# ylab-hi/BINARY

Measured on AMD Instinct MI355X. Metric: interval-overlap queries/s, higher is better.
Workload: dtype u32

## Files before the change

### binary_amd/csrc/build.hip

```cpp
#include "common.h"
#include "wave_device.h"

namespace bivx {
namespace {

constexpr int kThreads = 256;

__device__ __forceinline__ uint32_t len_bin(uint32_t low, uint32_t high, uint32_t &len) {
  len = high >= low ? high - low : 0u;
  return len == 0 ? 0u : 32u - (uint32_t)__clz((int)len);
}


constexpr uint32_t kStatsLdsEntries = 3300;
#ifndef BIVX_STATS_PARTS
#define BIVX_STATS_PARTS 64
#endif
constexpr uint32_t kStatsAutoParts = BIVX_STATS_PARTS;
#ifndef BIVX_STATS_THREADS
#define BIVX_STATS_THREADS 1024
#endif
constexpr int kStatsThreads = BIVX_STATS_THREADS;
#ifndef BIVX_STATS_UNROLL
#define BIVX_STATS_UNROLL 8
// ... 533 lines not shown
            const uint32_t g = atomicAdd(ngaps, 1u);
            if (g < gap_cap) gaps[g] = Gap{g0, gc, gv, 0u};
          }
        } else {
          for (uint32_t c = lane; c < gc; c += kWave) table[g0 + c] = gv;
        }
      }
    };
    cooperative(cnt > kInlineFill, e0, cnt, val);
    cooperative(tcnt > kInlineFill, t0, tcnt, tval);
  }
}

__global__ __launch_bounds__(kThreads) void k_fill_gaps(const Gap *__restrict__ gaps, const uint32_t *__restrict__ ngaps,
                                                        uint32_t gap_cap, uint32_t *__restrict__ table) {
  const uint32_t ng = min(*ngaps, gap_cap);
  const uint32_t t = blockIdx.x * kThreads + threadIdx.x, nt = gridDim.x * kThreads;
  for (uint32_t g = 0; g < ng; ++g) {
    const Gap gp = gaps[g];
    for (uint32_t c = t; c < gp.count; c += nt) table[gp.first + c] = gp.value;
  }
}

__global__ __launch_bounds__(kThreads) void k_max_cell(uint32_t *__restrict__ table, size_t nentries,
                                                       uint32_t *__restrict__ out) {
  uint32_t m = 0;
  auto diff = [](uint32_t a, uint32_t b) { return b > a ? b - a : 0u; };
  const size_t n4 = nentries ? (nentries - 1) / 4 : 0;
  const uint4 *t4 = reinterpret_cast<const uint4 *>(table);
  const size_t stride = (size_t)gridDim.x * kThreads;
  for (size_t g = (size_t)blockIdx.x * kThreads + threadIdx.x; g < n4; g += 2 * stride) {
    const size_t g2 = g + stride;
    const bool two = g2 < n4;
    const uint4 v = t4[g];
    const uint32_t nx = table[4 * g + 4];
    uint4 w = make_uint4(0u, 0u, 0u, 0u);
    uint32_t nw = 0;
    if (two) {
      w = t4[g2];
      nw = table[4 * g2 + 4];
    }
    m = max(max(m, diff(v.x, v.y)), max(max(diff(v.y, v.z), diff(v.z, v.w)), diff(v.w, nx)));
    if (two) m = max(max(m, diff(w.x, w.y)), max(max(diff(w.y, w.z), diff(w.z, w.w)), diff(w.w, nw)));
  }
  if (blockIdx.x == 0)
    for (size_t i = 4 * n4 + threadIdx.x; i + 1 < nentries; i += kThreads) m = max(m, diff(table[i], table[i + 1]));
  if (blockIdx.x == 0 && threadIdx.x < 3) table[nentries + threadIdx.x] = 0xFFFFFFFFu;
  block_max_to(m, out);
}

__global__ __launch_bounds__(kThreads) void k_self_queries(const uint2 *__restrict__ se, const SegDesc *__restrict__ seg,
                                                           const uint32_t *__restrict__ seg_chrom, uint32_t nseg, size_t n,
                                                           uint32_t *__restrict__ qchrom, uint32_t *__restrict__ qlow,
                                                           uint32_t *__restrict__ qhigh) {
  const size_t i = (size_t)blockIdx.x * kThreads + threadIdx.x;
  if (i >= n) return;
  uint32_t lo = 0, hi = nseg;
  while (hi - lo > 1) {
    const uint32_t m = (lo + hi) >> 1;
    if ((size_t)seg[m].begin <= i) lo = m; else hi = m;
  }
  const uint2 e = se[i];
  qchrom[i] = seg_chrom[lo];
  qlow[i] = e.x;
  qhigh[i] = e.y;
}

inline unsigned grid_for(size_t n, int per_block, unsigned cap = 0) {
  size_t nb = (n + (size_t)per_block - 1) / (size_t)per_block;
  if (nb < 1) nb = 1;
  if (cap && nb > cap) nb = cap;
// ... 112 lines not shown
  for (int shift = first_shift; shift < nbits || iota; shift += kRadixBits) {
    if (!(hist0_ready && shift == first_shift))
      hipLaunchKernelGGL(k_radix_hist, dim3(nblocks), dim3(kSortThreads), 0, s, *keys, n, shift, hist, nblocks);
    hipLaunchKernelGGL(k_radix_rows, dim3(kRadix), dim3(kThreads), 0, s, hist, offs, totals, nblocks);
    if (iota)
      hipLaunchKernelGGL(k_radix_scatter<true>, dim3(nblocks), dim3(kSortThreads), 0, s, *keys, *vals, *keys_alt,
                         *vals_alt, n, shift, offs, totals, nblocks);
    else
      hipLaunchKernelGGL(k_radix_scatter<false>, dim3(nblocks), dim3(kSortThreads), 0, s, *keys, *vals, *keys_alt,
                         *vals_alt, n, shift, offs, totals, nblocks);
    BIVX_HIP(hipGetLastError());
    iota = false;
    uint32_t *t = *keys; *keys = *keys_alt; *keys_alt = t;
    t = *vals; *vals = *vals_alt; *vals_alt = t;
  }
  return 0;
}

size_t finalize_gap_capacity(uint64_t nentries, uint32_t nseg) { return (size_t)(nentries / kCoopMax) + 2u * nseg + 64u; }
size_t finalize_gap_bytes(uint64_t nentries, uint32_t nseg) { return finalize_gap_capacity(nentries, nseg) * sizeof(Gap); }

int launch_finalize(const uint32_t *d_keys, const uint32_t *d_ids, const uint32_t *d_low, const uint32_t *d_high,
                    const SegDesc *d_seg, const uint2 *d_segkey, uint32_t nseg, uint2 *d_se, uint2 *d_rec,
                    uint32_t *d_table, uint64_t nentries, void *d_gaps, uint32_t *d_ngaps, uint32_t *d_max_cell,
                    size_t n, hipStream_t s) {
  if (n == 0 || nseg == 0) return 0;
  const uint32_t nchunks = grid_for(n, kThreads * kFinSlots);
  const unsigned grid = ((nchunks + 7u) / 8u) * 8u;
  const uint32_t cap = (uint32_t)finalize_gap_capacity(nentries, nseg);
  Gap *gaps = static_cast<Gap *>(d_gaps);
  if (d_keys)
    hipLaunchKernelGGL(k_finalize<true>, dim3(grid), dim3(kThreads), 0, s, d_keys, d_ids, d_low, d_high, d_seg, d_segkey, nseg,
                       d_se, d_rec, d_table, gaps, d_ngaps, cap, n, nchunks);
  else
    hipLaunchKernelGGL(k_finalize<false>, dim3(grid), dim3(kThreads), 0, s, d_keys, d_ids, d_low, d_high, d_seg, d_segkey,
                       nseg, d_se, d_rec, d_table, gaps, d_ngaps, cap, n, nchunks);
  hipLaunchKernelGGL(k_fill_gaps, dim3(256), dim3(kThreads), 0, s, gaps, d_ngaps, cap, d_table);
  hipLaunchKernelGGL(k_max_cell, dim3(grid_for(nentries, kThreads * 8, 512)), dim3(kThreads), 0, s, d_table, (size_t)nentries,
                     d_max_cell);
  BIVX_HIP(hipGetLastError());
  return 0;
}

int launch_self_queries(const uint2 *d_se, const SegDesc *d_seg, const uint32_t *d_seg_chrom, uint32_t nseg, size_t n,
                        uint32_t *d_qchrom, uint32_t *d_qlow, uint32_t *d_qhigh, hipStream_t s) {
  if (n == 0 || nseg == 0) return 0;
  hipLaunchKernelGGL(k_self_queries, dim3(grid_for(n, kThreads)), dim3(kThreads), 0, s, d_se, d_seg, d_seg_chrom, nseg, n,
                     d_qchrom, d_qlow, d_qhigh);
  BIVX_HIP(hipGetLastError());
  return 0;
}

int launch_gather_intervals(const uint32_t *d_chrom, const uint32_t *d_low, const uint32_t *d_high,
                            const uint32_t *d_ids, size_t n, size_t n_intervals, uint32_t *d_c, uint32_t *d_l,
                            uint32_t *d_h, hipStream_t s) {
  if (n == 0) return 0;
  hipLaunchKernelGGL(k_gather_intervals, dim3(grid_for(n, kThreads)), dim3(kThreads), 0, s, d_chrom, d_low, d_high,
                     d_ids, n, n_intervals, d_c, d_l, d_h);
  BIVX_HIP(hipGetLastError());
  return 0;
}

// ... 2 lines not shown
```

### binary_amd/csrc/capi.hip

```cpp
#include <algorithm>
#include <atomic>
#include <chrono>
#include <cstdarg>
#include <cstdio>
#include <cstdlib>
#include <condition_variable>
#include <cstring>
#include <map>
#include <mutex>
#include <new>
#include <unordered_map>
#include <unordered_set>
#include <vector>

#include "common.h"

namespace bivx {

static thread_local char g_err[512] = "";

void set_error(const char *fmt, ...) {
  va_list ap;
  va_start(ap, fmt);
  vsnprintf(g_err, sizeof(g_err), fmt, ap);
// ... 16 lines not shown
    void *p = nullptr;
    size_t cap = 0;
  };
  DevBuf b_se, b_table, b_seg;
  DevBuf b_keys[2], b_ids[2];
  DevBuf b_misc, b_radix, b_scalar, b_segof;
  DevBuf b_astats;
  bool astats_ready = false;
  size_t astats_n = 0;
  hipEvent_t astats_ev = nullptr;
  uint32_t *h_scalars = nullptr;
  void *h_stage = nullptr;
  size_t h_stage_cap = 0;
  std::vector<hipEvent_t> ev_pending, ev_free;
  mutable DevBuf b_selfq;
  mutable bool selfq_valid = false;
  mutable std::mutex self_mutex;
  uint32_t *d_seg_chrom = nullptr;
  bool built = false;
  uint2 *d_se = nullptr;
  uint2 *d_rec = nullptr;
  uint32_t *d_id = nullptr;
  uint32_t *d_table = nullptr;
  SegDesc *d_seg = nullptr;
  uint2 *d_chrom_rng = nullptr;
  uint32_t nchrom = 0, nseg = 0, ntypes = 1;
  std::vector<uint32_t> max_segs;
  uint64_t nentries = 0;
  uint32_t max_cell = 0;
  uint32_t max_window = 0;
  uint32_t order_shift = 0;
  size_t built_n = 0;
  double build_ms = 0.0;
  struct Workspace {
    void *p = nullptr;
    bool needs_reset = false;
    void *self_p = nullptr;
    size_t self_cap = 0;
  };
  mutable std::mutex ws_mutex;
  mutable std::unordered_map<hipStream_t, Workspace> ws_of_stream;
  mutable std::unordered_set<hipStream_t> reader_streams;
  uint32_t *h_err = nullptr;
  uint32_t *d_err = nullptr;
  mutable std::atomic<uint64_t> errors_reported{0};
  mutable std::mutex cache_mutex;
// ... 96 lines not shown
    if (!p) BIVX_HIP(dev_malloc(&p, bytes));
    ptrs.emplace_back(p, bytes);
    *out = static_cast<T *>(p);
    return 0;
  }
  void release(void *p) {
    for (auto &q : ptrs)
      if (q.first == p) q.first = nullptr;
  }
};

void drop_block_cache(const bivx_index *idx) {
  std::lock_guard<std::mutex> lock(idx->cache_mutex);
  for (auto &kv : idx->cache_free) (void)hipFree(kv.second);
  idx->cache_free.clear();
  idx->cache_bytes = 0;
}

void free_built(bivx_index *idx) {
  idx->d_se = nullptr;
  idx->d_rec = nullptr;
  idx->d_id = nullptr;
  idx->d_table = nullptr;
  idx->d_seg = nullptr;
  idx->d_chrom_rng = nullptr;
  idx->nchrom = idx->nseg = 0;
  idx->ntypes = 1;
  idx->max_segs.clear();
  idx->nentries = 0;
  idx->built = false;
  idx->selfq_valid = false;
}

void release_build_blocks(bivx_index *idx) {
  for (bivx_index::DevBuf *b : {&idx->b_se, &idx->b_table, &idx->b_seg, &idx->b_keys[0],
                                &idx->b_keys[1], &idx->b_ids[0], &idx->b_ids[1], &idx->b_misc, &idx->b_radix, &idx->b_scalar, &idx->b_segof, &idx->b_selfq, &idx->b_astats}) {
    (void)hipFree(b->p);
    b->p = nullptr;
    b->cap = 0;
  }
}

int ensure_block(bivx_index::DevBuf &b, size_t bytes) {
  if (bytes <= b.cap && b.p) return 0;
  (void)hipFree(b.p);
  b.p = nullptr;
// ... 297 lines not shown
      (void)packed_span;
    }
  }
  return 0;
}

int bits_for(uint32_t maxval) {
  int b = 0;
  while (maxval) {
    ++b;
    maxval >>= 1;
  }
  return b;
}

static thread_local uint32_t *g_lane_d_err = nullptr;

IndexView view_of(const bivx_index *idx, uint32_t svtype = 0) {
  IndexView v;
  v.se = idx->d_se;
  v.rec = idx->d_rec;
  v.id = idx->d_id;
  v.table = idx->d_table;
  v.seg = idx->d_seg;
  const uint32_t row = svtype < idx->ntypes ? svtype : idx->ntypes;
  v.chrom_rng = idx->d_chrom_rng + (size_t)row * idx->nchrom;
  v.nchrom = idx->nchrom;
  v.nseg = idx->nseg;
  v.max_segs = row < idx->max_segs.size() ? idx->max_segs[row] : 0;
  v.nslots = idx->built_n < 0xFFFFFFFFull ? (uint32_t)idx->built_n : 0xFFFFFFFFu;
  v.max_cell = idx->max_cell;
  v.max_window = idx->max_window;
  v.order_shift = idx->order_shift;
  v.flt_kind = BIVX_FILTER_NONE;
  v.flt_dist = 0;
  v.flt_strand = 0;
  v.flt_qaux = nullptr;
  v.flt_iaux = nullptr;
  v.err = g_lane_d_err ? g_lane_d_err : idx->d_err;
  return v;
}

int report_device_errors(const bivx_index *idx, const char *who, uint32_t *block = nullptr) {
  uint32_t *e = block ? block : idx->h_err;
  if (__atomic_load_n(&e[kErrTimeout], __ATOMIC_RELAXED) == 0 && __atomic_load_n(&e[kErrWorkspace], __ATOMIC_RELAXED) == 0)
    return 0;
// ... 493 lines not shown
    const uint32_t *cs = plan.chrom_seg.data() + (size_t)c * ntypes;
    rng[c] = make_uint2(cs[0], cs[ntypes] - cs[0]);
    max_segs[0] = std::max(max_segs[0], cs[ntypes] - cs[0]);
    for (uint32_t t = 1; t < ntypes; ++t) {
      rng[(size_t)t * nchrom + c] = make_uint2(cs[t], cs[t + 1] - cs[t]);
      max_segs[t] = std::max(max_segs[t], cs[t + 1] - cs[t]);
    }
  }
  if (!plan.bin2seg.empty()) std::memcpy(hm + off_b2s, plan.bin2seg.data(), plan.bin2seg.size() * sizeof(uint32_t));
  BIVX_HIP(hipMemcpyAsync(dm, hm, meta_bytes, hipMemcpyHostToDevice, s));

  uint32_t max_cell = 0, order_shift = 0;
  if (n) {
    for (int k = 0; k < 2; ++k) {
      BIVX_TRY(ensure_block(idx->b_keys[k], n * 4));
      BIVX_TRY(ensure_block(idx->b_ids[k], (n + 2) * 4));
    }
    BIVX_TRY(ensure_block(idx->b_radix, std::max(radix_scratch_bytes(n), finalize_gap_bytes(plan.nentries, nseg))));
    const bool dense = plan.key_span <= 0xFFFFFFFFull && !std::getenv("BIVX_BUILD_TWO_STAGE");
    const size_t se_bytes = ((n + 2) * sizeof(uint2) + 255) & ~(size_t)255;
    BIVX_TRY(ensure_block(idx->b_se, 2 * se_bytes));
    idx->d_se = static_cast<uint2 *>(idx->b_se.p);
    idx->d_rec = reinterpret_cast<uint2 *>(static_cast<char *>(idx->b_se.p) + se_bytes);
    BIVX_TRY(ensure_block(idx->b_table, ((size_t)plan.nentries + 3) * 4));
    idx->d_table = static_cast<uint32_t *>(idx->b_table.p);
    auto sort_and_finalize = [&](int skip) -> int {
      uint32_t *kA = static_cast<uint32_t *>(idx->b_keys[0].p), *kB = static_cast<uint32_t *>(idx->b_keys[1].p);
      uint32_t *vA = static_cast<uint32_t *>(idx->b_ids[0].p), *vB = static_cast<uint32_t *>(idx->b_ids[1].p);
      if (dense) {
        BIVX_TRY(launch_make_keys(kBuildKeyDense, idx->d_chrom, d_type, ntypes, idx->d_low, idx->d_high, n, d_bin2seg, d_segkey,
                                  nullptr, nullptr, kA, idx->b_radix.p, s, skip));
        BIVX_TRY(radix_sort_pairs(&kA, &vA, &kB, &vB, n, bits_for((uint32_t)(plan.key_span - 1)), idx->b_radix.p, true, true, s,
                                  skip));
      } else {
        BIVX_TRY(ensure_block(idx->b_segof, n * 4));
        uint32_t *d_seg_of = static_cast<uint32_t *>(idx->b_segof.p);
        BIVX_TRY(launch_make_keys(kBuildKeyLow, idx->d_chrom, d_type, ntypes, idx->d_low, idx->d_high, n, d_bin2seg, d_segkey,
                                  nullptr, d_seg_of, kA, idx->b_radix.p, s));
        BIVX_TRY(radix_sort_pairs(&kA, &vA, &kB, &vB, n, bits_for(plan.max_low), idx->b_radix.p, true, true, s));
        if (nseg > 1) {
          BIVX_TRY(launch_make_keys(kBuildKeySegOfId, idx->d_chrom, d_type, ntypes, idx->d_low, idx->d_high, n, d_bin2seg,
                                    d_segkey, vA, d_seg_of, kA, nullptr, s));
          BIVX_TRY(radix_sort_pairs(&kA, &vA, &kB, &vB, n, bits_for(nseg - 1), idx->b_radix.p, false, false, s));
        }
      }
      idx->d_id = vA;
      BIVX_TRY(launch_finalize(dense ? kA : nullptr, idx->d_id, idx->d_low, idx->d_high, idx->d_seg, d_segkey, nseg, idx->d_se,
                               idx->d_rec, idx->d_table, plan.nentries, idx->b_radix.p, d_scalar + 3, d_scalar + 2, n, s));
      BIVX_HIP(hipMemcpyAsync(idx->h_scalars + 2, d_scalar + 2, 4, hipMemcpyDeviceToHost, s));
      return 0;
    };
    int skip = dense ? (int)plan.order_shift : 0;
    BIVX_TRY(sort_and_finalize(skip));
    if (skip > 0) {
      BIVX_HIP(hipStreamSynchronize(s));
      if (hs[2] > kCrowdedCell) {
        BIVX_HIP(hipMemsetAsync(d_scalar + 2, 0, 8, s));
        skip = 0;
        BIVX_TRY(sort_and_finalize(0));
      }
    }
    order_shift = (uint32_t)skip;
  }
  BIVX_HIP(hipStreamSynchronize(s));
  if (n) max_cell = hs[2];
  idx->nchrom = nchrom;
  idx->nseg = nseg;
  idx->ntypes = ntypes;
  idx->max_segs = std::move(max_segs);
  idx->nentries = plan.nentries;
  idx->max_cell = max_cell;
// ... 280 lines not shown
    return BIVX_E_INVALID;
  }
  BIVX_NOT_SHARDED(idx, "bivx_stream_status");
  BIVX_GUARD(idx);
  BIVX_HIP(hipStreamSynchronize(static_cast<hipStream_t>(stream)));
  return report_device_errors(idx, "bivx_stream_status");
}

int bivx_debug_corrupt_workspace(const bivx_index *idx, void *stream) {
  if (!idx) {
    set_error("bivx_debug_corrupt_workspace: null index");
    return BIVX_E_INVALID;
  }
  BIVX_NOT_SHARDED(idx, "bivx_debug_corrupt_workspace");
  BIVX_GUARD(idx);
  hipStream_t s = static_cast<hipStream_t>(stream);
  std::lock_guard<std::mutex> lock(idx->ws_mutex);
  auto it = idx->ws_of_stream.find(s);
  if (it == idx->ws_of_stream.end()) {
    set_error("bivx_debug_corrupt_workspace: no workspace for this stream yet");
    return BIVX_E_STATE;
  }
  BIVX_HIP(hipMemsetAsync(it->second.p, 0x7F, sizeof(uint32_t), s));
  return 0;
}

const char *bivx_query_kernel_name(const bivx_index *idx, size_t q, uint64_t hit_capacity, int sort_by_id,
                                   const bivx_filter *filter) {
  if (!idx || idx->sharded || !idx->built) return "";
  IndexView view;
  if (view_with_filter(idx, filter, view) != 0) return "";
  if (pipe_eligible(view, q, hit_capacity, sort_by_id != 0, false)) return "k_query_pipe";
  const bool ms = pipe_ms_eligible(view, q, hit_capacity, false);
  if (pipe_dense_eligible(view, q, hit_capacity, sort_by_id != 0, false))
    return ms ? "k_query_pipe_dense|k_query_pipe_ms" : "k_query_pipe_dense|k_query_fused";
  return ms ? "k_query_pipe_ms" : "k_query_fused";
}

int bivx_sort_hits_dev(const bivx_index *idx, const uint64_t *d_offsets, uint32_t *d_hit_ids, size_t q, void *stream) {
  if (!idx || (q && !d_offsets)) {
    set_error("bivx_sort_hits_dev: null argument");
    return BIVX_E_INVALID;
  }
  BIVX_NOT_SHARDED(idx, "bivx_sort_hits_dev");
  BIVX_GUARD(idx);
  return launch_sort_hits(d_offsets, d_hit_ids, q, ~0ull, static_cast<hipStream_t>(stream));
// ... 375 lines not shown
    set_error("bivx_query_sharded_dev: not a sharded handle (bivx_create_sharded); a single-device index answers "
              "device-resident batches with bivx_query_dev_s");
    return BIVX_E_STATE;
  }
  return sharded_query_dev(idx->sharded, qchrom, qlow, qhigh, q, sort_by_id, out);
}

int bivx_get_stats(const bivx_index *idx, bivx_stats *out) {
  if (!idx || !out) {
    set_error("bivx_get_stats: null argument");
    return BIVX_E_INVALID;
  }
  if (idx->sharded) {
    sharded_stats(idx->sharded, out);
    return 0;
  }
  memset(out, 0, sizeof(*out));
  out->n_intervals = idx->n;
  out->n_chroms = idx->nchrom;
  out->n_segments = idx->nseg;
  out->n_cells = idx->nentries;
  out->staging_bytes = (uint64_t)idx->cap * 12;
  if (idx->built)
    out->index_bytes = (uint64_t)idx->built_n * 20 + idx->nentries * 4 + (uint64_t)idx->nseg * sizeof(SegDesc) +
                       ((uint64_t)idx->nchrom + 1) * 4;
  out->build_ms = idx->build_ms;
  {
    volatile uint32_t *e = idx->h_err;
    out->prefix_timeouts = idx->errors_reported.load() + ((e[kErrTimeout] | e[kErrWorkspace]) ? 1u : 0u);
  }
  return 0;
}

}
```

### binary_amd/csrc/common.h

```cpp
#pragma once

#include <hip/hip_runtime.h>

#include <cstddef>
#include <cstdint>

#include "../../include/bivx.h"

namespace bivx {

void set_error(const char *fmt, ...) __attribute__((format(printf, 1, 2)));

#define BIVX_HIP(call)                                                                              \
  do {                                                                                              \
    hipError_t bivx_e_ = (call);                                                                    \
    if (bivx_e_ != hipSuccess) {                                                                    \
      ::bivx::set_error("%s failed: %s (%s:%d)", #call, hipGetErrorString(bivx_e_), __FILE__,       \
                        __LINE__);                                                                  \
      return BIVX_E_HIP;                                                                            \
    }                                                                                               \
  } while (0)

#define BIVX_TRY(call)              \
  do {                              \
    int bivx_rc_ = (call);          \
    if (bivx_rc_ != 0) return bivx_rc_; \
  } while (0)

constexpr int kWave = 64;
constexpr int kLenBins = 33;

struct SegDesc {
  uint32_t begin, end;
  uint32_t base, last;
  uint32_t shift;
  uint32_t table_off;
  uint32_t maxlen;
  uint32_t ncell;
};
static_assert(sizeof(SegDesc) == 32, "SegDesc layout");
constexpr uint32_t kSegPacked = 1u << 8;

struct IndexView {
  const uint2 *se;
  const uint2 *rec;
  const uint32_t *id;
  const uint32_t *table;
  const SegDesc *seg;
  const uint2 *chrom_rng;
  uint32_t nchrom;
  uint32_t nseg;
  uint32_t max_segs;
  uint32_t nslots;
  uint32_t max_cell;
  uint32_t max_window;
  uint32_t order_shift;
  uint32_t flt_kind;
  uint32_t flt_dist;
  uint32_t flt_strand;
  const uint32_t *flt_qaux;
  const uint32_t *flt_iaux;
  uint32_t *err;
};
constexpr uint32_t kErrTimeout = 0;
constexpr uint32_t kErrWorkspace = 1;
constexpr uint32_t kErrWords = 16;

struct BinStats {
  uint32_t count;
  uint32_t min_low;
  uint32_t max_low;
  uint32_t max_len;
  uint32_t n_inverted;
};

struct ShardedState;
int sharded_create(ShardedState **out, const int *devices, int ndev);
void sharded_destroy(ShardedState *st);
int sharded_num_devices(const ShardedState *st);
int sharded_device_of_chrom(const ShardedState *st, uint32_t chrom);
int sharded_append(ShardedState *st, const uint32_t *chrom, const uint32_t *low, const uint32_t *high,
                   const uint8_t *svtype, size_t n);
int sharded_clear(ShardedState *st);
size_t sharded_size(const ShardedState *st);
bool sharded_is_built(const ShardedState *st);
uint32_t sharded_num_chroms(const ShardedState *st);
// ... 27 lines not shown
int launch_bin_stats(const uint32_t *d_chrom, const uint8_t *d_type, uint32_t ntypes, const uint32_t *d_low,
                     const uint32_t *d_high, size_t n, uint32_t nparts, BinStats *d_stats, hipStream_t s);
uint32_t bin_stats_auto_parts();
int launch_bin_stats_auto(const uint32_t *d_chrom, const uint32_t *d_low, const uint32_t *d_high, size_t n, BinStats *d_stats,
                          uint32_t *d_scal, hipStream_t s);
size_t auto_stats_bytes();
int launch_init_auto_stats(void *d_block, hipStream_t s);
int launch_append_stats(const uint32_t *d_chrom, const uint32_t *d_low, const uint32_t *d_high, size_t n, uint32_t *d_out_chrom,
                        uint32_t *d_out_low, uint32_t *d_out_high, void *d_block, hipStream_t s);
int launch_max_chrom_type(const uint32_t *d_chrom, const uint8_t *d_type, size_t n, uint32_t *d_out2, hipStream_t s);
int launch_gather_u8(const uint8_t *d_src, const uint32_t *d_ids, size_t n, size_t n_src, uint8_t *d_out,
                     hipStream_t s);
enum : int { kBuildKeyDense = 0, kBuildKeyLow = 1, kBuildKeySegOfId = 2 };
int launch_make_keys(int mode, const uint32_t *d_chrom, const uint8_t *d_type, uint32_t ntypes, const uint32_t *d_low,
                     const uint32_t *d_high, size_t n, const uint32_t *d_bin2seg, const uint2 *d_segkey,
                     const uint32_t *d_ids, uint32_t *d_seg_of, uint32_t *d_keys, void *d_hist0, hipStream_t s,
                     int first_shift = 0);
size_t radix_scratch_bytes(size_t n);
int radix_sort_pairs(uint32_t **keys, uint32_t **vals, uint32_t **keys_alt, uint32_t **vals_alt, size_t n,
                     int nbits, void *d_scratch, bool vals_are_iota, bool hist0_ready, hipStream_t s, int first_shift = 0);
size_t finalize_gap_bytes(uint64_t nentries, uint32_t nseg);
int launch_finalize(const uint32_t *d_keys, const uint32_t *d_ids, const uint32_t *d_low, const uint32_t *d_high,
                    const SegDesc *d_seg, const uint2 *d_segkey, uint32_t nseg, uint2 *d_se, uint2 *d_rec,
                    uint32_t *d_table, uint64_t nentries, void *d_gaps, uint32_t *d_ngaps, uint32_t *d_max_cell,
                    size_t n, hipStream_t s);
int launch_gather_intervals(const uint32_t *d_chrom, const uint32_t *d_low, const uint32_t *d_high,
                            const uint32_t *d_ids, size_t n, size_t n_intervals, uint32_t *d_c, uint32_t *d_l,
                            uint32_t *d_h, hipStream_t s);
int launch_self_queries(const uint2 *d_se, const SegDesc *d_seg, const uint32_t *d_seg_chrom, uint32_t nseg, size_t n,
                        uint32_t *d_qchrom, uint32_t *d_qlow, uint32_t *d_qhigh, hipStream_t s);

int launch_query_tiny(const IndexView &v, const uint32_t *d_qchrom, const uint32_t *d_qlow, const uint32_t *d_qhigh,
                      size_t q, uint64_t *d_offsets, uint32_t *d_hits, uint64_t cap, hipStream_t s);
int launch_fill(const IndexView &v, const uint32_t *d_qchrom, const uint32_t *d_qlow, const uint32_t *d_qhigh,
                size_t q, const uint64_t *d_offsets, uint32_t *d_hits, hipStream_t s);
int launch_any(const IndexView &v, const uint32_t *d_qchrom, const uint32_t *d_qlow, const uint32_t *d_qhigh,
               size_t q, uint32_t *d_first, hipStream_t s);
int launch_sort_hits(const uint64_t *d_offsets, uint32_t *d_hits, size_t q, uint64_t cap, hipStream_t s,
                     const uint32_t *d_cond = nullptr, uint32_t seq = 0, uint64_t total_hint = 0);
size_t fused_workspace_bytes(size_t q);
int launch_query_fused(const IndexView &v, const uint32_t *d_qchrom, const uint32_t *d_qlow,
                       const uint32_t *d_qhigh, size_t q, uint64_t *d_offsets, uint32_t *d_hits, uint64_t cap,
                       void *d_ws, bool self_clean, bool sort_ids, hipStream_t s, uint32_t *d_counts = nullptr,
                       uint64_t *d_total = nullptr);

bool pipe_eligible(const IndexView &v, size_t q, uint64_t cap, bool sort_ids, bool unordered);
size_t pipe_queries_per_launch();
size_t pipe_ms_queries_per_launch();
// ... 21 lines not shown
```

### binary_amd/csrc/query_pipe.hip

```cpp
#include <atomic>
#include <cstdlib>

#include "prefix_device.h"
#include "query_device.h"

namespace bivx {
namespace {

#ifndef BIVX_PIPE_THREADS
#define BIVX_PIPE_THREADS 1024
#endif
constexpr int kPThreads = BIVX_PIPE_THREADS;
constexpr int kPWaves = kPThreads / kWave;
constexpr int kWorkers = kPWaves - 1;
constexpr uint32_t kPTile = kWorkers * kWave;
constexpr uint32_t kRing = 8;
#ifndef BIVX_DEFER
#define BIVX_DEFER 2
#endif
#ifndef BIVX_WSLEEP
#define BIVX_WSLEEP 16
#endif
#ifndef BIVX_SSLEEP
#define BIVX_SSLEEP 2
// ... 77 lines not shown

__device__ __forceinline__ uint32_t lds_load(const uint32_t *p) {
  return __hip_atomic_load(p, __ATOMIC_ACQUIRE, __HIP_MEMORY_SCOPE_WORKGROUP);
}
__device__ __forceinline__ void lds_store(uint32_t *p, uint32_t x) {
  __hip_atomic_store(p, x, __ATOMIC_RELEASE, __HIP_MEMORY_SCOPE_WORKGROUP);
}
__device__ __forceinline__ void lds_wait_eq(const uint32_t *p, uint32_t x) {
  while (lds_load(p) != x) __builtin_amdgcn_s_sleep(BIVX_WSLEEP);
}

__device__ __forceinline__ void stage_to_output(const uint32_t *stage, uint32_t *out, uint32_t n, uint32_t lane) {
  typedef uint32_t u32x4_a16 __attribute__((ext_vector_type(4)));
  const uint32_t n4 = n & ~3u;
  for (uint32_t i = lane * 4u; i < n4; i += kWave * 4u)
    __builtin_nontemporal_store(*reinterpret_cast<const u32x4_a16 *>(stage + i), reinterpret_cast<u32x4_a4 *>(out + i));
  if (n4 + lane < n) stream_store(out + n4 + lane, stage[n4 + lane]);
}

struct Win {
  uint32_t a, b, base;
  uint32_t fl;
};

template <uint32_t KEEP>
__device__ __forceinline__ uint32_t eval16(const char *rb, uint32_t p0, uint32_t plast, uint32_t wm16, uint32_t base,
                                           uint32_t qh, uint32_t ql, uint32_t *keep, uint32_t &kpos) {
  uint4 r[8];
#pragma unroll
  for (uint32_t j = 0; j < 8; ++j)
#ifdef BIVX_EXP_MAXLOADS
    if (p0 + j <= plast && j < BIVX_EXP_MAXLOADS) r[j] = *reinterpret_cast<const uint4 *>(rb + ((p0 + j) << 4));
#else
    if (p0 + j <= plast) r[j] = *reinterpret_cast<const uint4 *>(rb + ((p0 + j) << 4));
#endif
  uint32_t m = 0;
#pragma unroll
  for (uint32_t j = 0; j < 8; ++j) {
    const uint32_t rr[2] = {r[j].x, r[j].z};
#pragma unroll
    for (uint32_t k = 0; k < 2; ++k) {
      const uint32_t rl = (rr[k] - base) & 0xFFFFu;
      m = shift_in_le_ge(m, rl, qh, rl + (rr[k] >> 16), ql);
    }
  }
  m = (__brev(m) >> 16) & wm16;
// ... 400 lines not shown
  }

  auto tid = [] {
    uint32_t t = threadIdx.x;
    asm volatile("" : "+v"(t));
    return t;
  };
  auto kept_slots = [&] {
    const uint32_t t = tid();
    return reinterpret_cast<uint32_t *>(&s_keep[(t & ~(uint32_t)(kWave - 1)) * (kPKeep / 4)]) + (t & (kWave - 1));
  };
  auto slab_of_wave = [&] { return &s_keep[(tid() & ~(uint32_t)(kWave - 1)) * (kPKeep / 4)]; };

  auto query_of = [&](uint32_t t) {
    kargs_t p = fresh(ka);
    const size_t q = p->a.q_begin + (size_t)t * kPTile + threadIdx.x;
    IndexView w;
    w.nchrom = p->v.nchrom;
    w.flt_qaux = nullptr;
    return load_query<false>(w, cs, p->a.qchrom, p->a.qlow, p->a.qhigh, q, t < p->a.ntiles && q < p->a.q_end);
  };

  auto window_of = [&](const Query &q) {
    Win w{0u, 0u, 0u, 0u};
    if (q.nseg) {
      const SegDesc d = load_seg(segs + q.s0);
      const uint32_t x = q.lo > d.maxlen ? q.lo - d.maxlen : 0u;
      if (!(q.hi < d.base || x > d.last || q.hi < x)) {
        const uint32_t sh = d.shift & 31u;
        const uint32_t ca = x <= d.base ? 0u : (x - d.base) >> sh;
        const uint32_t cb = q.hi >= d.last ? d.ncell : ((q.hi - d.base) >> sh) + 1u;
        const char *t = reinterpret_cast<const char *>(fresh(ka)->v.table);
        w.a = *reinterpret_cast<const uint32_t *>(t + ((d.table_off + ca) << 2));
        w.b = *reinterpret_cast<const uint32_t *>(t + ((d.table_off + cb) << 2));
        w.base = d.base + (ca << sh);
        w.fl = 1u | ((d.shift & kSegPacked) != 0 && ((uint64_t)(cb - ca) << sh) <= 65536ull ? 2u : 0u);
      }
    }
    return w;
  };

  struct Pending {
    bool have, staged;
    uint32_t tile, wtotal, state;
  };
  Pending pd_[kDefer];
#pragma unroll
  for (uint32_t k = 0; k < kDefer; ++k) pd_[k] = Pending{false, false, 0u, 0u, 0u};
  auto flush = [&](const Pending &pd, uint32_t j) {
    TileSlot &os = s_slot[j % kRing];
    uint32_t *const stage = s_stage[wave][j % kDefer];
    lds_wait_eq(&os.gen_base, j + 1);
    const uint64_t wpos0 = os.base + os.wbase[wave];
    kargs_t p = fresh(ka);
    const size_t q_end = p->a.q_end;
    const size_t q = p->a.q_begin + (size_t)pd.tile * kPTile + threadIdx.x;
    uint64_t *off = p->a.offsets;
    if (pd.staged) {
      if (q < q_end) {
// ... 13 lines not shown
    } else {
      const uint64_t lp = (uint64_t)stage[3 * lane] | (uint64_t)stage[3 * lane + 1] << 32;
      const uint32_t c = stage[3 * lane + 2];
      if (q < q_end) {
        off[q] = wpos0 + lp;
        uint32_t *counts = p->a.counts;
        if (counts) counts[q] = c;
        if (q == q_end - 1) *(counts ? p->a.total_out : off + q_end) = wpos0 + lp + c;
      }
      if (lane == 0 && p->a.cap != 0) {
        uint64_t *ws = p->a.ws;
        uint32_t *todo = reinterpret_cast<uint32_t *>(ws + kWsList);
        todo[atomicAdd(reinterpret_cast<unsigned int *>(ws + kWsTodo), 1u)] = pd.tile * 16u + (uint32_t)wave;
      }
    }
    wave_sync_lds();
    if (lane == 0) __hip_atomic_fetch_add(&os.flushed, 1u, __ATOMIC_RELEASE, __HIP_MEMORY_SCOPE_WORKGROUP);
  };

  lds_wait_eq(&s_slot[0].gen_ticket, 1u);
  if (threadIdx.x == 0) { WGSTAMP(2); }
  uint32_t tile = __builtin_amdgcn_readfirstlane(s_slot[0].tile);
  uint32_t qlo, qhi;
  Win wn;
  {
    const Query q0 = query_of(tile);
    qlo = q0.lo;
    qhi = q0.hi;
    wn = window_of(q0);
  }
  if (threadIdx.x == 0) { WGSTAMP(3); }

  for (uint32_t it = 0;; ++it) {
    const bool live = tile < A(ntiles);
    int path = 0;
    uint32_t qw_a = 0;
    uint32_t m32 = 0, lbase = 0;
    uint32_t kinfo = 0;
    uint32_t cnt = 0, loff = 0, wtotal = 0;
    bool staged = false, no_ids = false;
    uint64_t lpos64 = 0;
    if (live) {
      PSTAMP(tile, 0);
      const bool nonempty = (wn.fl & 1u) != 0 && wn.b > wn.a;
      const uint32_t al = wn.a & ~1u;
      qw_a = wn.a;
      path = 0;
      if (!__any(nonempty && !((wn.fl & 2u) != 0 && wn.b - al < 32u))) {
        lbase = wave_min(nonempty ? al : 0xFFFFFFFFu);
        const bool in_slab = nonempty && wn.b - lbase <= kPKeep * (kWave / 2);
        const uint32_t nin = (uint32_t)__popcll(__ballot(in_slab)), nne = (uint32_t)__popcll(__ballot(nonempty));
        path = nin >= kSlabMinLanes && nin == nne ? 1 : 2;
        if (path == 2 && (BIVX_EXP & 8) == 0 &&
            !__any(nonempty && (wn.b - al > 16u || (qlo > wn.base && qlo - wn.base > 0xFFFFu) || (al >> 1) >= (1u << 26))))
          path = 3;
      }
      no_ids = A(cap) == 0;
      if (path == 1) {
        const uint32_t npairs = (wave_max(nonempty ? wn.b : 0u) - lbase + 1u) >> 1;
        const uint4 *src = reinterpret_cast<const uint4 *>(fresh(ka)->v.rec) + (lbase >> 1);
        uint4 *const slab = slab_of_wave();
        for (uint32_t i = tid() & (kWave - 1); i < npairs; i += kWave) slab[i] = src[i];
        wave_sync_lds();
        const Window w{wn.a, wn.b, wn.base, 1u, true};
        m32 = slab_mask32(slab, lbase, w, qlo, qhi, nonempty);
        cnt = (uint32_t)__popc(m32);
      } else if (path == 3) {
        wtotal = coop_place16(fresh(ka)->v.rec, reinterpret_cast<uint32_t *>(slab_of_wave()), wn, nonempty, qlo, qhi,
                              tid() & (kWave - 1), !no_ids, cnt, loff);
      } else if (path == 2) {
#ifdef BIVX_NO_COOP
        m32 = lanes_mask32<kPKeep>(fresh(ka)->v.rec, wn, nonempty, qlo, qhi, kept_slots());
        kinfo = 0xFFFFFFFFu;
#else
        m32 = coop_mask32<kPKeep>(fresh(ka)->v.rec, reinterpret_cast<uint32_t *>(slab_of_wave()), wn, nonempty, qlo, qhi,
                                  tid() & (kWave - 1), kinfo);
#endif
        cnt = (uint32_t)__popc(m32);
      } else {
        kargs_t p = fresh(ka);
        IndexView v1;
        v1.se = p->v.se;
        v1.rec = p->v.rec;
        v1.id = p->v.id;
        v1.table = p->v.table;
        v1.seg = nullptr;
        v1.chrom_rng = nullptr;
        v1.nchrom = 0;
        v1.nseg = 0;
        v1.max_segs = 1;
        v1.flt_kind = BIVX_FILTER_NONE;
        v1.flt_dist = 0;
        v1.flt_strand = 0;
        v1.flt_qaux = nullptr;
        v1.flt_iaux = nullptr;
        v1.order_shift = p->v.order_shift;
        v1.err = nullptr;
        const Query qy = query_of(tile);
        cnt = enumerate_hits<Mode::Count, false, false, kPKeep, kRows, false>(v1, segs, qy, nullptr, 0, 0, nullptr);
      }
      bool huge = false;
      if (path != 3) {
        const uint32_t incl = wave_scan_incl(cnt);
        loff = incl - cnt;
        huge = __any(cnt >= (1u << 22));
        wtotal = wave_last(incl);
      }
      staged = !huge && (no_ids ? wtotal < 65536u : path != 0 && wtotal <= kPStage);
      uint64_t wt64 = wtotal;
      lpos64 = loff;
      if (huge) {
        uint64_t i64 = cnt;
#pragma unroll
        for (int d = 1; d < kWave; d <<= 1) {
          const uint64_t o = __shfl_up((unsigned long long)i64, d, kWave);
          if (lane >= d) i64 += o;
        }
        lpos64 = i64 - cnt;
        wt64 = __shfl((unsigned long long)i64, kWave - 1, kWave);
      }
      TileSlot &sl = s_slot[it % kRing];
      if (lane == 0) {
        sl.wsum[wave] = wt64;
        __hip_atomic_fetch_add(&sl.arrived, 1u, __ATOMIC_RELEASE, __HIP_MEMORY_SCOPE_WORKGROUP);
      }
      PSTAMP(tile, 1);
    }

    uint32_t ntile = 0xFFFFFFFFu;
    Query nqy{0u, 0u, 0u, 0u, 0u};
    if (live) {
      TileSlot &nx = s_slot[(it + 1) % kRing];
      lds_wait_eq(&nx.gen_ticket, it + 2);
      ntile = __builtin_amdgcn_readfirstlane(nx.tile);
      nqy = query_of(ntile);
      PSTAMP(tile, 2);
    }

    if (pd_[kDefer - 1].have) flush(pd_[kDefer - 1], it - kDefer);
    if (!live) {
#pragma unroll
      for (uint32_t k = kDefer - 1; k-- > 0;)
        if (pd_[k].have) flush(pd_[k], it - 1 - k);
      if (threadIdx.x == 0) {
        WGSTAMP(4);
        WGSTAMP_VAL(6, (unsigned long long)it);
      }
      break;
    }
    PSTAMP(tile, 3);
    const Win nwn = window_of(nqy);

#pragma unroll
    for (uint32_t k = kDefer - 1; k > 0; --k) pd_[k] = pd_[k - 1];
    pd_[0] = Pending{true, staged, tile, wtotal, (loff << 16) | cnt};
    uint32_t *const stage = s_stage[wave][it % kDefer];
    if (!staged) {
      stage[3 * lane] = (uint32_t)lpos64;
      stage[3 * lane + 1] = (uint32_t)(lpos64 >> 32);
      stage[3 * lane + 2] = cnt;
    } else if ((BIVX_EXP & 1) != 0) {
    } else if (!no_ids && path == 1) {
      const uint2 *s2 = reinterpret_cast<const uint2 *>(slab_of_wave()) + ((qw_a & ~1u) - lbase);
      uint32_t *dst = stage + loff;
      while (m32) {
        const uint32_t j = (uint32_t)__ffs((int)m32) - 1u;
        m32 &= m32 - 1u;
        *dst++ = s2[j].y;
      }
    } else if (!no_ids && path == 3) {
      const uint4 *src = reinterpret_cast<const uint4 *>(slab_of_wave());
      uint4 *dst = reinterpret_cast<uint4 *>(stage);
      for (uint32_t i = tid() & (kWave - 1); i < (wtotal + 3u) >> 2; i += kWave) dst[i] = src[i];
    } else if (!no_ids && path == 2) {
// ... 47 lines not shown
        BIVX_SORT8(0, 1, 2, 3, 4, 5, 6, 7)
        BIVX_SORT8(15, 14, 13, 12, 11, 10, 9, 8)
#pragma unroll
        for (uint32_t d = 8; d > 0; d >>= 1)
#pragma unroll
          for (uint32_t i = 0; i < 16u; ++i)
            if ((i & d) == 0) BIVX_CE(i, i + d)
#pragma unroll
        for (uint32_t k = 0; k < 16u; ++k)
          if (k < cnt) stage[loff + k] = x[k];
#undef BIVX_SORT8
#undef BIVX_CE
      } else if (cnt > 16u) {
        uint32_t *const tmp = reinterpret_cast<uint32_t *>(slab_of_wave());
        rank_sort_list<8>(stage, tmp, loff, cnt);
        for (uint32_t k = 0; k < cnt; ++k) stage[loff + k] = tmp[loff + k];
      }
    }
    wave_sync_lds();
    PSTAMP(tile, 4);
    tile = ntile;
    qlo = nqy.lo;
    qhi = nqy.hi;
    wn = nwn;
  }

}

constexpr uint32_t kDRound = 2 * kPStage;

__global__ __launch_bounds__(kPThreads, 8) void k_query_pipe_dense(IndexView v_in, PipeArgs a_in) {
  (void)v_in;
  (void)a_in;
  kargs_t ka = (kargs_t)__builtin_amdgcn_kernarg_segment_ptr();
  __shared__ SegDesc s_seg[kLdsSegs];
  __shared__ uint2 s_cs[kLdsChroms];
  __shared__ TileSlot s_slot[kRing];
  __shared__ uint4 s_keep[kWorkers * kWave * (kPKeep / 4)];
  __shared__ __attribute__((aligned(16))) uint32_t s_stage[kWorkers][2 * kPStage];
  {
    kargs_t p = fresh(ka);
    const uint32_t w = __hip_atomic_load(reinterpret_cast<const uint32_t *>(p->a.ws + kWsOrder), __ATOMIC_RELAXED,
                                         __HIP_MEMORY_SCOPE_AGENT);
    if (w != p->a.seq && !(p->a.flags & kFlagSorted)) return;
  }
  const int lane = threadIdx.x & (kWave - 1);
  const int wave = threadIdx.x >> 6;
// ... 177 lines not shown
      in_slab_path = !__any(!fits);
      if (in_slab_path) {
        if (__any(nonempty)) {
          npairs = (wave_max(nonempty ? wn.b : 0u) - lbase + 1u) >> 1;
        } else {
          lbase = 0;
        }
        const uint4 *src = reinterpret_cast<const uint4 *>(fresh(ka)->v.rec) + (lbase >> 1);
        uint4 *const slab = slab_of_wave();
        for (uint32_t i = tid() & (kWave - 1); i < npairs; i += kWave) slab[i] = src[i];
        wave_sync_lds();
        const Window w{wn.a, wn.b, wn.base, 1u, true};
        const bool short32 = !__any(nonempty && wn.b - al >= 32u);
        mask = short32 ? (uint64_t)slab_mask32(slab, lbase, w, qlo, qhi, nonempty)
                       : slab_mask64(slab, lbase, w, qlo, qhi, nonempty);
        cnt = (uint32_t)__popcll(mask);
      } else {
        kargs_t p = fresh(ka);
        IndexView v1;
        v1.se = p->v.se;
        v1.rec = p->v.rec;
        v1.id = p->v.id;
        v1.table = p->v.table;
        v1.seg = nullptr;
        v1.chrom_rng = nullptr;
        v1.nchrom = 0;
        v1.nseg = 0;
        v1.max_segs = 1;
        v1.nslots = 0;
        v1.flt_kind = BIVX_FILTER_NONE;
        v1.flt_dist = 0;
        v1.flt_strand = 0;
        v1.flt_qaux = nullptr;
        v1.flt_iaux = nullptr;
        v1.order_shift = p->v.order_shift;
        v1.err = nullptr;
        const Query qy = query_of(tile);
        cnt = enumerate_hits<Mode::Count, false, false, kPKeep, kRows, false>(v1, segs, qy, nullptr, 0, 0, nullptr);
      }
      const uint32_t incl = wave_scan_incl(cnt);
      loff = incl - cnt;
      const bool huge = __any(cnt >= (1u << 22));
      wtotal = wave_last(incl);
      uint64_t wt64 = wtotal;
      lpos64 = loff;
      if (huge) {
// ... 399 lines not shown
      if (!live) {
        if (pa.have) flush(pa, it - 1);
        break;
      }
    } else {
      if (pa.have) flush(pa, it - 1);
      if (!live) break;
    }
    bool too_long;
    uint32_t cnt;
    const bool no_ids = A(cap) == 0 || !keep_mode;
    if (no_ids)
      cnt = group_scan<kMsCount, F>(ka, segs, qy, true, nullptr, 0u, 0u, (uint32_t)lane, s_stage[wave] + kMsDefer * kMsKeepWords, too_long);
    else
      cnt = group_scan<kMsKeep, F>(ka, segs, qy, true, s_stage[wave] + (kMsDefer == 2 ? (it & 1u) * kMsKeepWords : 0u), 0u, 0u, (uint32_t)lane,
                                   s_stage[wave] + kMsDefer * kMsKeepWords, too_long);
    if (too_long) {
      kargs_t p = fresh(ka);
      IndexView v1;
      v1.se = p->v.se;
      v1.rec = p->v.rec;
      v1.id = p->v.id;
      v1.table = p->v.table;
      v1.seg = nullptr;
      v1.chrom_rng = nullptr;
      v1.nchrom = 0;
      v1.nseg = 0;
      v1.max_segs = p->v.max_segs;
      v1.nslots = 0;
      v1.max_cell = 0;
      v1.max_window = 0;
      v1.flt_kind = p->v.flt_kind;
      v1.flt_dist = p->v.flt_dist;
      v1.flt_strand = p->v.flt_strand;
      v1.flt_qaux = nullptr;
      v1.flt_iaux = p->v.flt_iaux;
      v1.order_shift = p->v.order_shift;
      v1.err = nullptr;
      cnt = enumerate_hits<Mode::Count, F, true, kKeep, kRows, false>(v1, segs, qy, nullptr, 0, 0, nullptr);
    }
    const uint32_t incl = wave_scan_incl(cnt);
    const bool huge = __any(cnt >= (1u << 22));
    const bool general = too_long || huge;
    const uint32_t pair_cnt = cnt + (uint32_t)__builtin_amdgcn_ds_swizzle((int)cnt, 0x041F);
    const bool fits = !general && !__any(pair_cnt > 2u * kMsKeepN);
    const bool kept = fits && !no_ids;
// ... 509 lines not shown
```

Before: 36.99 billion.

## Add compressed delta table for window lookups in query pipeline

Builds a compressed companion to the cell table: for each group of 8 entries it stores a base value plus seven 4-bit deltas, or an escape marker pointing back to the full table. The query pipeline's window lookup now loads these 8-byte group descriptors and decodes the boundaries with a udot8 instruction, instead of reading two raw table entries. The intent is to shrink the footprint of the random table probes so they hit cache more often. In exchange it adds decode ALU work, an extra dependent load on the escape path, and a larger k_max_cell build pass. It also adds a test-only verification kernel.

```diff
diff --git a/binary_amd/csrc/build.hip b/binary_amd/csrc/build.hip
--- a/binary_amd/csrc/build.hip
+++ b/binary_amd/csrc/build.hip
@@ -579,31 +579,70 @@
   }
 }
 
+__device__ __forceinline__ uint2 dirc_group(const uint32_t (&t)[8], size_t g) {
+  uint32_t steps = 0;
+  bool esc = false;
+#pragma unroll
+  for (int i = 0; i < 7; ++i) {
+    const uint32_t d = t[i + 1] - t[i];
+    esc |= t[i + 1] < t[i] || d > 15u;
+    steps |= (d & 15u) << (4 * i);
+  }
+  return make_uint2(t[0], esc ? kDircEscape | (uint32_t)g : steps);
+}
+
 __global__ __launch_bounds__(kThreads) void k_max_cell(uint32_t *__restrict__ table, size_t nentries,
-                                                       uint32_t *__restrict__ out) {
+                                                       uint32_t *__restrict__ out, uint2 *__restrict__ dirc) {
   uint32_t m = 0;
   auto diff = [](uint32_t a, uint32_t b) { return b > a ? b - a : 0u; };
-  const size_t n4 = nentries ? (nentries - 1) / 4 : 0;
+  auto group = [&](const uint4 v, const uint4 w, uint32_t nx, size_t g) {
+    const uint32_t t[8] = {v.x, v.y, v.z, v.w, w.x, w.y, w.z, w.w};
+#pragma unroll
+    for (int i = 0; i < 7; ++i) m = max(m, diff(t[i], t[i + 1]));
+    m = max(m, diff(t[7], nx));
+    dirc[g] = dirc_group(t, g);
+  };
+  const size_t n8 = nentries ? (nentries - 1) / 8 : 0;
   const uint4 *t4 = reinterpret_cast<const uint4 *>(table);
   const size_t stride = (size_t)gridDim.x * kThreads;
-  for (size_t g = (size_t)blockIdx.x * kThreads + threadIdx.x; g < n4; g += 2 * stride) {
+  for (size_t g = (size_t)blockIdx.x * kThreads + threadIdx.x; g < n8; g += 2 * stride) {
     const size_t g2 = g + stride;
-    const bool two = g2 < n4;
-    const uint4 v = t4[g];
-    const uint32_t nx = table[4 * g + 4];
-    uint4 w = make_uint4(0u, 0u, 0u, 0u);
-    uint32_t nw = 0;
+    const bool two = g2 < n8;
+    const uint4 v = t4[2 * g], w = t4[2 * g + 1];
+    const uint32_t nx = table[8 * g + 8];
+    uint4 v2 = make_uint4(0u, 0u, 0u, 0u), w2 = v2;
+    uint32_t nx2 = 0;
     if (two) {
-      w = t4[g2];
-      nw = table[4 * g2 + 4];
-    }
-    m = max(max(m, diff(v.x, v.y)), max(max(diff(v.y, v.z), diff(v.z, v.w)), diff(v.w, nx)));
-    if (two) m = max(max(m, diff(w.x, w.y)), max(max(diff(w.y, w.z), diff(w.z, w.w)), diff(w.w, nw)));
-  }
-  if (blockIdx.x == 0)
-    for (size_t i = 4 * n4 + threadIdx.x; i + 1 < nentries; i += kThreads) m = max(m, diff(table[i], table[i + 1]));
+      v2 = t4[2 * g2];
+      w2 = t4[2 * g2 + 1];
+      nx2 = table[8 * g2 + 8];
+    }
+    group(v, w, nx, g);
+    if (two) group(v2, w2, nx2, g2);
+  }
+  if (blockIdx.x == 0) {
+    for (size_t i = 8 * n8 + threadIdx.x; i + 1 < nentries; i += kThreads) m = max(m, diff(table[i], table[i + 1]));
+    const size_t g = n8 + threadIdx.x;
+    if (g < dirc_groups(nentries)) {
+      uint32_t t[8];
+      t[0] = table[8 * g];
+#pragma unroll
+      for (int i = 1; i < 8; ++i) t[i] = 8 * g + i < nentries ? table[8 * g + i] : t[i - 1];
+      dirc[g] = dirc_group(t, g);
+    }
+  }
   if (blockIdx.x == 0 && threadIdx.x < 3) table[nentries + threadIdx.x] = 0xFFFFFFFFu;
   block_max_to(m, out);
+}
+
+__global__ __launch_bounds__(kThreads) void k_check_dirc(const uint32_t *__restrict__ table, const uint2 *__restrict__ dirc,
+                                                         size_t nentries, unsigned long long *__restrict__ out) {
+  for (size_t e = (size_t)blockIdx.x * kThreads + threadIdx.x; e < nentries; e += (size_t)gridDim.x * kThreads) {
+    const uint2 g = dirc[e >> kDircShift];
+    const uint32_t k = (uint32_t)e & ((1u << kDircShift) - 1u);
+    if (dirc_entry(g, k, table) != table[e]) atomicAdd(&out[0], 1ull);
+    if (k == 0 && (g.y & kDircEscape)) atomicAdd(&out[1], 1ull);
+  }
 }
 
 __global__ __launch_bounds__(kThreads) void k_self_queries(const uint2 *__restrict__ se, const SegDesc *__restrict__ seg,
@@ -762,8 +801,8 @@
 
 int launch_finalize(const uint32_t *d_keys, const uint32_t *d_ids, const uint32_t *d_low, const uint32_t *d_high,
                     const SegDesc *d_seg, const uint2 *d_segkey, uint32_t nseg, uint2 *d_se, uint2 *d_rec,
-                    uint32_t *d_table, uint64_t nentries, void *d_gaps, uint32_t *d_ngaps, uint32_t *d_max_cell,
-                    size_t n, hipStream_t s) {
+                    uint32_t *d_table, uint2 *d_dirc, uint64_t nentries, void *d_gaps, uint32_t *d_ngaps,
+                    uint32_t *d_max_cell, size_t n, hipStream_t s) {
   if (n == 0 || nseg == 0) return 0;
   const uint32_t nchunks = grid_for(n, kThreads * kFinSlots);
   const unsigned grid = ((nchunks + 7u) / 8u) * 8u;
@@ -776,8 +815,16 @@
     hipLaunchKernelGGL(k_finalize<false>, dim3(grid), dim3(kThreads), 0, s, d_keys, d_ids, d_low, d_high, d_seg, d_segkey,
                        nseg, d_se, d_rec, d_table, gaps, d_ngaps, cap, n, nchunks);
   hipLaunchKernelGGL(k_fill_gaps, dim3(256), dim3(kThreads), 0, s, gaps, d_ngaps, cap, d_table);
-  hipLaunchKernelGGL(k_max_cell, dim3(grid_for(nentries, kThreads * 8, 512)), dim3(kThreads), 0, s, d_table, (size_t)nentries,
-                     d_max_cell);
+  hipLaunchKernelGGL(k_max_cell, dim3(grid_for(nentries, kThreads * 16, 512)), dim3(kThreads), 0, s, d_table, (size_t)nentries,
+                     d_max_cell, d_dirc);
+  BIVX_HIP(hipGetLastError());
+  return 0;
+}
+
+int launch_check_dirc(const uint32_t *d_table, const uint2 *d_dirc, uint64_t nentries, uint64_t *d_out2, hipStream_t s) {
+  if (nentries == 0) return 0;
+  hipLaunchKernelGGL(k_check_dirc, dim3(grid_for(nentries, kThreads, 1024)), dim3(kThreads), 0, s, d_table, d_dirc,
+                     (size_t)nentries, reinterpret_cast<unsigned long long *>(d_out2));
   BIVX_HIP(hipGetLastError());
   return 0;
 }
diff --git a/binary_amd/csrc/capi.hip b/binary_amd/csrc/capi.hip
--- a/binary_amd/csrc/capi.hip
+++ b/binary_amd/csrc/capi.hip
@@ -62,6 +62,7 @@
   uint2 *d_rec = nullptr;
   uint32_t *d_id = nullptr;
   uint32_t *d_table = nullptr;
+  uint2 *d_dirc = nullptr;
   SegDesc *d_seg = nullptr;
   uint2 *d_chrom_rng = nullptr;
   uint32_t nchrom = 0, nseg = 0, ntypes = 1;
@@ -204,6 +205,7 @@
   idx->d_rec = nullptr;
   idx->d_id = nullptr;
   idx->d_table = nullptr;
+  idx->d_dirc = nullptr;
   idx->d_seg = nullptr;
   idx->d_chrom_rng = nullptr;
   idx->nchrom = idx->nseg = 0;
@@ -547,6 +549,7 @@
   v.rec = idx->d_rec;
   v.id = idx->d_id;
   v.table = idx->d_table;
+  v.dirc = idx->d_dirc;
   v.seg = idx->d_seg;
   const uint32_t row = svtype < idx->ntypes ? svtype : idx->ntypes;
   v.chrom_rng = idx->d_chrom_rng + (size_t)row * idx->nchrom;
@@ -1086,8 +1089,10 @@
     BIVX_TRY(ensure_block(idx->b_se, 2 * se_bytes));
     idx->d_se = static_cast<uint2 *>(idx->b_se.p);
     idx->d_rec = reinterpret_cast<uint2 *>(static_cast<char *>(idx->b_se.p) + se_bytes);
-    BIVX_TRY(ensure_block(idx->b_table, ((size_t)plan.nentries + 3) * 4));
+    const size_t table_bytes = (((size_t)plan.nentries + 3) * 4 + 255) & ~(size_t)255;
+    BIVX_TRY(ensure_block(idx->b_table, table_bytes + dirc_groups(plan.nentries) * sizeof(uint2)));
     idx->d_table = static_cast<uint32_t *>(idx->b_table.p);
+    idx->d_dirc = reinterpret_cast<uint2 *>(static_cast<char *>(idx->b_table.p) + table_bytes);
     auto sort_and_finalize = [&](int skip) -> int {
       uint32_t *kA = static_cast<uint32_t *>(idx->b_keys[0].p), *kB = static_cast<uint32_t *>(idx->b_keys[1].p);
       uint32_t *vA = static_cast<uint32_t *>(idx->b_ids[0].p), *vB = static_cast<uint32_t *>(idx->b_ids[1].p);
@@ -1110,7 +1115,8 @@
       }
       idx->d_id = vA;
       BIVX_TRY(launch_finalize(dense ? kA : nullptr, idx->d_id, idx->d_low, idx->d_high, idx->d_seg, d_segkey, nseg, idx->d_se,
-                               idx->d_rec, idx->d_table, plan.nentries, idx->b_radix.p, d_scalar + 3, d_scalar + 2, n, s));
+                               idx->d_rec, idx->d_table, idx->d_dirc, plan.nentries, idx->b_radix.p, d_scalar + 3, d_scalar + 2,
+                               n, s));
       BIVX_HIP(hipMemcpyAsync(idx->h_scalars + 2, d_scalar + 2, 4, hipMemcpyDeviceToHost, s));
       return 0;
     };
@@ -1437,6 +1443,36 @@
     return BIVX_E_STATE;
   }
   BIVX_HIP(hipMemsetAsync(it->second.p, 0x7F, sizeof(uint32_t), s));
+  return 0;
+}
+
+int bivx_test_check_dirc(const bivx_index *idx, uint64_t *out) {
+  if (!idx || !out) {
+    set_error("bivx_test_check_dirc: null argument");
+    return BIVX_E_INVALID;
+  }
+  BIVX_NOT_SHARDED(idx, "bivx_test_check_dirc");
+  if (!idx->built) {
+    set_error("bivx_test_check_dirc: index not built");
+    return BIVX_E_STATE;
+  }
+  BIVX_GUARD(idx);
+  BIVX_HIP(hipStreamSynchronize(idx->stream));
+  uint64_t *d = nullptr;
+  BIVX_HIP(hipMalloc(&d, 2 * sizeof(uint64_t)));
+  uint64_t h[2] = {0, 0};
+  int rc = hipMemsetAsync(d, 0, 2 * sizeof(uint64_t), idx->stream) == hipSuccess ? 0 : BIVX_E_HIP;
+  if (rc == 0 && idx->built_n) rc = launch_check_dirc(idx->d_table, idx->d_dirc, idx->nentries, d, idx->stream);
+  if (rc == 0 && hipMemcpyAsync(h, d, sizeof h, hipMemcpyDeviceToHost, idx->stream) != hipSuccess) rc = BIVX_E_HIP;
+  if (rc == 0 && hipStreamSynchronize(idx->stream) != hipSuccess) rc = BIVX_E_HIP;
+  (void)hipFree(d);
+  if (rc) {
+    set_error("bivx_test_check_dirc: device error");
+    return rc;
+  }
+  out[0] = h[0];
+  out[1] = h[1];
+  out[2] = idx->built_n ? dirc_groups(idx->nentries) : 0;
   return 0;
 }
 
@@ -1858,7 +1894,8 @@
   out->n_cells = idx->nentries;
   out->staging_bytes = (uint64_t)idx->cap * 12;
   if (idx->built)
-    out->index_bytes = (uint64_t)idx->built_n * 20 + idx->nentries * 4 + (uint64_t)idx->nseg * sizeof(SegDesc) +
+    out->index_bytes = (uint64_t)idx->built_n * 20 + idx->nentries * 4 + dirc_groups(idx->nentries) * sizeof(uint2) +
+                       (uint64_t)idx->nseg * sizeof(SegDesc) +
                        ((uint64_t)idx->nchrom + 1) * 4;
   out->build_ms = idx->build_ms;
   {
diff --git a/binary_amd/csrc/common.h b/binary_amd/csrc/common.h
--- a/binary_amd/csrc/common.h
+++ b/binary_amd/csrc/common.h
@@ -46,6 +46,7 @@
   const uint2 *rec;
   const uint32_t *id;
   const uint32_t *table;
+  const uint2 *dirc;
   const SegDesc *seg;
   const uint2 *chrom_rng;
   uint32_t nchrom;
@@ -62,6 +63,19 @@
   const uint32_t *flt_iaux;
   uint32_t *err;
 };
+
+constexpr uint32_t kDircShift = 3;
+constexpr uint32_t kDircEscape = 1u << 31;
+__host__ __device__ inline size_t dirc_groups(uint64_t nentries) { return (size_t)((nentries + 7) >> kDircShift); }
+
+__device__ __forceinline__ uint32_t dirc_entry_plain(uint2 g, uint32_t k) {
+  return g.x + __builtin_amdgcn_udot8(g.y & ((1u << (4u * k)) - 1u), 0x11111111u, 0u, false);
+}
+__device__ __forceinline__ uint32_t dirc_entry(uint2 g, uint32_t k, const uint32_t *table) {
+  if (g.y & kDircEscape) return table[((g.y & ~kDircEscape) << kDircShift) + k];
+  return dirc_entry_plain(g, k);
+}
+
 constexpr uint32_t kErrTimeout = 0;
 constexpr uint32_t kErrWorkspace = 1;
 constexpr uint32_t kErrWords = 16;
@@ -135,8 +149,9 @@
 size_t finalize_gap_bytes(uint64_t nentries, uint32_t nseg);
 int launch_finalize(const uint32_t *d_keys, const uint32_t *d_ids, const uint32_t *d_low, const uint32_t *d_high,
                     const SegDesc *d_seg, const uint2 *d_segkey, uint32_t nseg, uint2 *d_se, uint2 *d_rec,
-                    uint32_t *d_table, uint64_t nentries, void *d_gaps, uint32_t *d_ngaps, uint32_t *d_max_cell,
-                    size_t n, hipStream_t s);
+                    uint32_t *d_table, uint2 *d_dirc, uint64_t nentries, void *d_gaps, uint32_t *d_ngaps,
+                    uint32_t *d_max_cell, size_t n, hipStream_t s);
+int launch_check_dirc(const uint32_t *d_table, const uint2 *d_dirc, uint64_t nentries, uint64_t *d_out2, hipStream_t s);
 int launch_gather_intervals(const uint32_t *d_chrom, const uint32_t *d_low, const uint32_t *d_high,
                             const uint32_t *d_ids, size_t n, size_t n_intervals, uint32_t *d_c, uint32_t *d_l,
                             uint32_t *d_h, hipStream_t s);
diff --git a/binary_amd/csrc/query_pipe.hip b/binary_amd/csrc/query_pipe.hip
--- a/binary_amd/csrc/query_pipe.hip
+++ b/binary_amd/csrc/query_pipe.hip
@@ -123,6 +123,17 @@
   uint32_t a, b, base;
   uint32_t fl;
 };
+
+struct WinProbe {
+  uint2 ga, gb;
+  uint32_t base, fl;
+};
+__device__ __forceinline__ Win win_of(const WinProbe &p, const uint32_t *table) {
+  const uint32_t ka = (p.fl >> 2) & 7u, kb = (p.fl >> 5) & 7u;
+  if ((p.ga.y | p.gb.y) & kDircEscape)
+    return Win{dirc_entry(p.ga, ka, table), dirc_entry(p.gb, kb, table), p.base, p.fl & 3u};
+  return Win{dirc_entry_plain(p.ga, ka), dirc_entry_plain(p.gb, kb), p.base, p.fl & 3u};
+}
 
 template <uint32_t KEEP>
 __device__ __forceinline__ uint32_t eval16(const char *rb, uint32_t p0, uint32_t plast, uint32_t wm16, uint32_t base,
@@ -569,7 +580,7 @@
   };
 
   auto window_of = [&](const Query &q) {
-    Win w{0u, 0u, 0u, 0u};
+    WinProbe w{make_uint2(0u, 0u), make_uint2(0u, 0u), 0u, 0u};
     if (q.nseg) {
       const SegDesc d = load_seg(segs + q.s0);
       const uint32_t x = q.lo > d.maxlen ? q.lo - d.maxlen : 0u;
@@ -577,11 +588,13 @@
         const uint32_t sh = d.shift & 31u;
         const uint32_t ca = x <= d.base ? 0u : (x - d.base) >> sh;
         const uint32_t cb = q.hi >= d.last ? d.ncell : ((q.hi - d.base) >> sh) + 1u;
-        const char *t = reinterpret_cast<const char *>(fresh(ka)->v.table);
-        w.a = *reinterpret_cast<const uint32_t *>(t + ((d.table_off + ca) << 2));
-        w.b = *reinterpret_cast<const uint32_t *>(t + ((d.table_off + cb) << 2));
+        const uint32_t ea = d.table_off + ca, eb = d.table_off + cb;
+        const char *t = reinterpret_cast<const char *>(fresh(ka)->v.dirc);
+        w.ga = *reinterpret_cast<const uint2 *>(t + (ea & ~7u));
+        w.gb = *reinterpret_cast<const uint2 *>(t + (eb & ~7u));
         w.base = d.base + (ca << sh);
-        w.fl = 1u | ((d.shift & kSegPacked) != 0 && ((uint64_t)(cb - ca) << sh) <= 65536ull ? 2u : 0u);
+        w.fl = 1u | ((d.shift & kSegPacked) != 0 && ((uint64_t)(cb - ca) << sh) <= 65536ull ? 2u : 0u) | (ea & 7u) << 2 |
+               (eb & 7u) << 5;
       }
     }
     return w;
@@ -641,12 +654,12 @@
   if (threadIdx.x == 0) { WGSTAMP(2); }
   uint32_t tile = __builtin_amdgcn_readfirstlane(s_slot[0].tile);
   uint32_t qlo, qhi;
-  Win wn;
+  WinProbe wp;
   {
     const Query q0 = query_of(tile);
     qlo = q0.lo;
     qhi = q0.hi;
-    wn = window_of(q0);
+    wp = window_of(q0);
   }
   if (threadIdx.x == 0) { WGSTAMP(3); }
 
@@ -661,6 +674,7 @@
     uint64_t lpos64 = 0;
     if (live) {
       PSTAMP(tile, 0);
+      const Win wn = win_of(wp, fresh(ka)->v.table);
       const bool nonempty = (wn.fl & 1u) != 0 && wn.b > wn.a;
       const uint32_t al = wn.a & ~1u;
       qw_a = wn.a;
@@ -703,6 +717,7 @@
         v1.rec = p->v.rec;
         v1.id = p->v.id;
         v1.table = p->v.table;
+        v1.dirc = p->v.dirc;
         v1.seg = nullptr;
         v1.chrom_rng = nullptr;
         v1.nchrom = 0;
@@ -736,7 +751,7 @@
           if (lane >= d) i64 += o;
         }
         lpos64 = i64 - cnt;
-        wt64 = __shfl((unsigned long long)i64, kWave - 1, kWave);
+        wt64 = (uint64_t)wave_last((uint32_t)i64) | (uint64_t)wave_last((uint32_t)(i64 >> 32)) << 32;
       }
       TileSlot &sl = s_slot[it % kRing];
       if (lane == 0) {
@@ -768,7 +783,7 @@
       break;
     }
     PSTAMP(tile, 3);
-    const Win nwn = window_of(nqy);
+    const WinProbe nwp = window_of(nqy);
 
 #pragma unroll
     for (uint32_t k = kDefer - 1; k > 0; --k) pd_[k] = pd_[k - 1];
@@ -862,7 +877,7 @@
     tile = ntile;
     qlo = nqy.lo;
     qhi = nqy.hi;
-    wn = nwn;
+    wp = nwp;
   }
 
 }
@@ -1086,6 +1101,7 @@
         v1.rec = p->v.rec;
         v1.id = p->v.id;
         v1.table = p->v.table;
+        v1.dirc = p->v.dirc;
         v1.seg = nullptr;
         v1.chrom_rng = nullptr;
         v1.nchrom = 0;
@@ -1531,6 +1547,7 @@
       v1.rec = p->v.rec;
       v1.id = p->v.id;
       v1.table = p->v.table;
+      v1.dirc = p->v.dirc;
       v1.seg = nullptr;
       v1.chrom_rng = nullptr;
       v1.nchrom = 0;
```

Result: faster. 41.34 billion, median of 6 (+11.7%).
